# whwu95/MVFNet

Hardware: AMD Instinct MI355X
Metric: clips/sec (fwd+bwd) MVFNet-R50 8x8 224^2 (higher is better)
Workload: dtype bf16; 1 GPU; MVFNet-ResNet50 8x8, 32 clips/GPU of 8x3x224x224, bf16, train step: fwd (batch-stat BN) + loss + bwd + clip + SGD-nesterov; all through the HIP C ABI (stem + 16 bottlenecks + MVF + TSN head); clips_per_gpu=32, frames_per_clip=8, parallelism=dp1: replicas, one flat gradient all-reduce per step

## Files before the change

### include/mvfnet_hip.h

```cpp
#ifndef MVFNET_HIP_H
#define MVFNET_HIP_H

#include <stddef.h>
#include <stdint.h>

#ifdef __cplusplus
extern "C" {
#endif

#define MVF_ABI_VERSION 2

enum { MVF_OK = 0, MVF_EINVAL = -1, MVF_ESHAPE = -2, MVF_EWS = -3, MVF_EHIP = -4, MVF_EUNSUPPORTED = -5 };
enum { MVF_F32 = 0, MVF_BF16 = 1 };
enum { MVF_NCHW = 0, MVF_NHWC = 1 };
enum { MVF_VIEW_T = 1, MVF_VIEW_H = 2, MVF_VIEW_W = 4 };

int mvf_abi_version(void);
const char* mvf_last_error(void);

typedef struct {
    int32_t nt, c, h, w;
    int32_t n_segment;
    int32_t cs;
    int32_t mode;
// ... 158 lines not shown
                          int sums_rows, float* slabs, size_t slab_bytes, int dtype, void* stream);
int mvf_conv1x1_bnbwd_sums_pair(const void* a_in, int a_pitch, const void* w_a, const void* x_in, int x_pitch, const void* w_b, const void* g, int g_pitch,
                                const unsigned char* sign_bits, long m, int c, int k, const float* mean_a, const float* invstd_a, const float* mean_b,
                                const float* invstd_b, float* part_a, float* part_b, int rows, int dtype, void* stream);
int mvf_wgrad_slab_reduce(const float* slabs, int nsplit, int cout, int k, float* dw_oihw, void* stream);
int mvf_maxpool_bn_relu_fwd(const void* z, int n, int h, int w, int c, const float* scale, const float* shift, void* y,
                            unsigned char* argmax, int dtype, void* stream);
int mvf_maxpool_bn_relu_bwd(const unsigned char* argmax, const void* g, int n, int h, int w, int c, void* ga, int dtype,
                            void* stream);
int mvf_maxpool_bwd_sums_rows(int n, int h);
int mvf_maxpool_bn_relu_bwd_apply(const unsigned char* argmax, const void* g, int n, int h, int w, int c, const void* z, const float* gamma,
                                  const float* mean, const float* invstd, const float* scale, const float* shift, const float* dgamma,
                                  const float* dbeta, void* dz, int dtype, void* stream);
int mvf_maxpool_bn_relu_bwd_sums(const unsigned char* argmax, const void* g, int n, int h, int w, int c, void* ga, const void* z, const float* mean,
                                 const float* invstd, const float* scale, const float* shift, float* sums_part, int dtype, void* stream);
int mvf_head_train_fwd(const void* feat, int clips, int t, int hw, int c, const float* fc_w, const float* fc_b, int classes,
                       const long long* labels, const float* drop_mask ,
                       float* pooled, float* scores, float* dscores, float* loss_part, float* loss, int dtype, void* stream);
int mvf_ce_loss(const float* scores, const long long* labels, int clips, int classes, float* dscores, float* loss_part, float* loss,
                void* stream);
int mvf_head_train_bwd(const float* dscores, const float* pooled, const float* fc_w, const float* drop_mask, int clips, int t,
                       int hw, int c, int classes, float* dfc_w, float* dfc_b, float* dpool_ws , void* dfeat, int dtype,
                       void* stream);
size_t mvf_conv2d_wgrad_workspace_bytes(const mvf_conv_desc_t* d);
int mvf_conv2d_nhwc_wgrad(const mvf_conv_desc_t* d, const void* dz, const void* x, const void* x2, int kw_real,
                          int cin_real, int kw_packed, int cin_packed, float* dw_oihw, void* ws, size_t ws_bytes,
                          void* stream);
int mvf_conv2d_nhwc_wgrad_wgs(const mvf_conv_desc_t* d, const void* dz, const void* x, const void* x2, int kw_real,
                              int cin_real, int kw_packed, int cin_packed, float* dw_oihw, void* ws, size_t ws_bytes, int wgs, void* stream);
typedef struct {
// ... 51 lines not shown
```

### mvfnet_amd/_lib.py

```python
import ctypes as C
import os

import torch

_HERE = os.path.dirname(os.path.abspath(__file__))
LIB_PATH = os.environ.get("MVF_LIB_PATH") or os.path.join(_HERE, "libmvfnet_hip.so")

MVF_F32, MVF_BF16 = 0, 1
MVF_NCHW, MVF_NHWC = 0, 1
VIEW_T, VIEW_H, VIEW_W = 1, 2, 4
MODE_BITS = {"T": 1, "TH": 3, "THW": 7}
ERRNAMES = {-1: "MVF_EINVAL", -2: "MVF_ESHAPE", -3: "MVF_EWS", -4: "MVF_EHIP", -5: "MVF_EUNSUPPORTED"}


class MvfDesc(C.Structure):
    _fields_ = [("nt", C.c_int32), ("c", C.c_int32), ("h", C.c_int32), ("w", C.c_int32), ("n_segment", C.c_int32),
                ("cs", C.c_int32), ("mode", C.c_int32), ("layout", C.c_int32), ("dtype", C.c_int32)]


class ConvDesc(C.Structure):
    _fields_ = [("n", C.c_int32), ("h", C.c_int32), ("w", C.c_int32), ("cin", C.c_int32), ("cout", C.c_int32),
                ("kh", C.c_int32), ("kw", C.c_int32), ("stride", C.c_int32), ("pad", C.c_int32),
                ("ho", C.c_int32), ("wo", C.c_int32), ("x_pix_stride", C.c_int32),
                ("dtype", C.c_int32), ("relu", C.c_int32), ("split_c", C.c_int32), ("x2_pix_stride", C.c_int32), ("in_dil", C.c_int32),
# ... 130 lines not shown
    lib.mvf_bn_apply_bits.argtypes = [vp, i64, i32, fp, fp, vp, fp, fp, i32, vp, vp, i32, vp]
    lib.mvf_bn_bwd_apply_masked.restype = i32
    lib.mvf_bn_bwd_apply_masked.argtypes = [vp, i32, vp, vp, i64, i32, fp, fp, fp, fp, fp, fp, fp, i32, vp, i32, vp]
    lib.mvf_bn_bwd_reduce.restype = i32
    lib.mvf_bn_bwd_reduce.argtypes = [vp, i32, vp, vp, i64, i32, fp, fp, fp, fp, i32, vp, fp, fp, vp, sz, i32, vp]
    lib.mvf_bn_bwd_apply.restype = i32
    lib.mvf_bn_bwd_apply.argtypes = [vp, i32, vp, i64, i32, fp, fp, fp, fp, fp, fp, fp, i32, vp, i32, vp]
    lib.mvf_maxpool_bn_relu_fwd.restype = i32
    lib.mvf_maxpool_bn_relu_fwd.argtypes = [vp, i32, i32, i32, i32, fp, fp, vp, vp, i32, vp]
    lib.mvf_maxpool_bn_relu_bwd.restype = i32
    lib.mvf_maxpool_bn_relu_bwd.argtypes = [vp, vp, i32, i32, i32, i32, vp, i32, vp]
    lib.mvf_maxpool_bwd_sums_rows.restype = i32
    lib.mvf_maxpool_bwd_sums_rows.argtypes = [i32, i32]
    lib.mvf_maxpool_bn_relu_bwd_apply.restype = i32
    lib.mvf_maxpool_bn_relu_bwd_apply.argtypes = [vp, vp, i32, i32, i32, i32, vp, fp, fp, fp, fp, fp, fp, fp, vp, i32, vp]
    lib.mvf_maxpool_bn_relu_bwd_sums.restype = i32
    lib.mvf_maxpool_bn_relu_bwd_sums.argtypes = [vp, vp, i32, i32, i32, i32, vp, vp, fp, fp, fp, fp, fp, i32, vp]
    lib.mvf_head_train_fwd.restype = i32
    lib.mvf_head_train_fwd.argtypes = [vp, i32, i32, i32, i32, fp, fp, i32, ll, fp, fp, fp, fp, fp, fp, i32, vp]
    lib.mvf_conv2d_nhwc_fwd_mvf.restype = i32
    lib.mvf_conv2d_nhwc_fwd_mvf.argtypes = [cp, vp, vp, fp, fp, i32, i32, i32, vp, vp, sz, vp]
    lib.mvf_bn_bwd_pair.restype = i32
    lib.mvf_bn_bwd_pair.argtypes = [vp, i32, vp, vp, vp, i64, i32, fp, fp, fp, fp, fp, fp, fp, fp, fp, fp, vp, vp, vp, sz, i32, vp]
    lib.mvf_bn_bwd_wgrad_splits.restype = i32
    lib.mvf_bn_bwd_wgrad_splits.argtypes = [i64, i32, i32, i32, i32]
    lib.mvf_bn_bwd_wgrad_slab_bytes.restype = sz
    lib.mvf_bn_bwd_wgrad_slab_bytes.argtypes = [i64, i32, i32, i32, i32]
    lib.mvf_bn_bwd_apply_wgrad.restype = i32
    lib.mvf_bn_bwd_apply_wgrad.argtypes = [vp, i32, vp, vp, i64, i32, fp, fp, fp, fp, fp, fp, fp, i32, vp, vp, i32, i32, fp, sz, i32, vp]
    lib.mvf_bn_bwd_pair_wgrad.restype = i32
# ... 58 lines not shown
```

### mvfnet_amd/csrc/common.h

```cpp
#pragma once
#include <hip/hip_runtime.h>
#include <stdlib.h>
#include <string.h>
#include <strings.h>
#include <stdint.h>
#include <stdio.h>

#include "mvfnet_hip.h"

void mvf_set_error(const char* fmt, ...);

#define MVF_HIP_OK(call)                                                                        \
    do {                                                                                        \
        hipError_t e__ = (call);                                                                \
        if (e__ != hipSuccess) {                                                                \
            mvf_set_error("%s:%d: %s -> %s", __FILE__, __LINE__, #call, hipGetErrorString(e__)); \
            return MVF_EHIP;                                                                    \
        }                                                                                       \
    } while (0)

#define MVF_REQUIRE(cond, code, ...)    \
    do {                                \
        if (!(cond)) {                  \
            mvf_set_error(__VA_ARGS__); \
// ... 38 lines not shown
                       __uint_as_float(r.y << 16), __uint_as_float(r.y & 0xffff0000u));
}
__device__ __forceinline__ void st4(float* p, float4 v) { *reinterpret_cast<float4*>(p) = v; }
__device__ __forceinline__ void st4(bf16_t* p, float4 v) {
    uint2 r;
    r.x = pack_bf16x2(v.x, v.y);
    r.y = pack_bf16x2(v.z, v.w);
    *reinterpret_cast<uint2*>(p) = r;
}

__device__ __forceinline__ float hswish_f(float u) { return u * fminf(fmaxf(u + 3.0f, 0.0f), 6.0f) * (1.0f / 6.0f); }
__device__ __forceinline__ float hswish_grad_f(float u) {
    float r6 = fminf(fmaxf(u + 3.0f, 0.0f), 6.0f);
    float inner = (u > -3.0f && u < 3.0f) ? 1.0f : 0.0f;
    return r6 * (1.0f / 6.0f) + u * inner * (1.0f / 6.0f);
}

static inline size_t align_up(size_t v, size_t a) { return (v + a - 1) / a * a; }

static inline bool mvf_policy_lookup(const char* name, long* out) {
    const char* p = getenv("MVF_POLICY");
    if (!p) return false;
    const size_t n = strlen(name);
    while (*p) {
        while (*p == ',' || *p == ';' || *p == ' ') ++p;
        const char* e = p;
        while (*e && *e != ',' && *e != ';') ++e;
        const char* eq = (const char*)memchr(p, '=', (size_t)(e - p));
        if (eq && (size_t)(eq - p) == n && strncasecmp(p, name, n) == 0) {
            *out = strtol(eq + 1, nullptr, 10);
// ... 40 lines not shown
    const void* a;
    const void* w;
    const void* g;
    const unsigned char* bits;
    const float* c0;
    const float* c1;
    float* part;
    int rows, mode, M, N, K, xps;
};
struct Wgrad3x3C64Args {
    const void* dz;
    const void* x;
    float* part;
    int N, H, W, xps, nwg;
};
struct WgradStemArgs {
    const void* dz;
    const void* x;
    float* part;
    int N, H, W, Ho, Wo, nwg;
};
namespace mvf_internal {
struct BnBwdWgradArgs {
    const void* g;
    const void* z[2];
    const void* bits;
    const float *gamma[2], *mean[2], *invstd[2], *dgamma[2], *dbeta[2];
    const float *scale, *shift;
    void* dz[2];
    const void* x[2];
    int xps[2];
    float* part[2];
    int g_pitch, M, C, K;
    int rows_per_split, nsplit, ctiles, ktiles;
};
// ... 19 lines not shown
    const float *mean_a, *invstd_a, *mean_b, *invstd_b;
    float *part_a, *part_b;
    int aps, xps, g_pitch, M, rows, rows_per_split, nsplit;
};
int pw_sums_pair_launch(const PwSumsPairArgs& a, hipStream_t st);
int pw_bwd_fused_plan(long m, int c, int k, int* rows_per_split);
int pw_bwd_fused_launch(const PwBwdFusedArgs& a, hipStream_t st);
bool bnbwd_wgrad_tile(int c, int k, int nbn, int mask_mode, int* ct, int* kt);
int bnbwd_wgrad_plan(long m, int c, int k, int nbn, int mask_mode, int* rows_per_split, int* ctiles, int* ktiles);
int bnbwd_wgrad_launch(const BnBwdWgradArgs& a, int nbn, int mask_mode, hipStream_t st);
int wgrad_slab_reduce_launch(const float* part, int nsplit, int cout, int k, float* dw_oihw, hipStream_t st);
bool wgrad3x3_c64_ok(int n, int h, int w, int xps);
int wgrad3x3_c64_wgs(int n, int h);
int wgrad3x3_c64_launch(const Wgrad3x3C64Args& a, hipStream_t st);
bool wgrad_stem_ok(int n, int h, int w, int ho, int wo);
int wgrad_stem_wgs(int n, int ho);
int wgrad_stem_launch(const WgradStemArgs& a, hipStream_t st);
int stem_direct_launch(const StemDirectArgs& a, hipStream_t st);
int conv3x3_c64_launch(const Conv3x3C64Args& a, hipStream_t st);
int pw_sums_launch(const PwSumsArgs& a, hipStream_t st);
}

#ifdef __HIPCC__
typedef int i32x4 __attribute__((ext_vector_type(4)));
__device__ __forceinline__ i32x4 rsrc_words(const void* base, unsigned nbytes) {
    const unsigned long p = (unsigned long)base;
    i32x4 r;
    r.x = __builtin_amdgcn_readfirstlane((int)(unsigned)p);
    r.y = __builtin_amdgcn_readfirstlane((int)((unsigned)(p >> 32) & 0xffffu));
    r.z = __builtin_amdgcn_readfirstlane((int)nbytes);
// ... 13 lines not shown
```

### mvfnet_amd/csrc/train_ops.hip

```cpp
#include <algorithm>
#include <math.h>
#include <stdlib.h>

#include "common.h"

namespace {

constexpr int kThreads = 256;

struct ColPlan {
    int cqb;
    int rl;
    int gx;
    int gy;
    int rows;
};

ColPlan col_plan(long M, int C, int vn = 4, int blocks = 2048) {
    ColPlan p;
    const int cq = C / vn;
    int cqb = 1;
    while (cqb < cq && cqb < 64) cqb <<= 1;
    p.cqb = cqb;
    p.rl = kThreads / cqb;
// ... 901 lines not shown
template <typename ET, int MODE>
__global__ __launch_bounds__(256) void maxpool_bn_bwd_blk_kernel(const unsigned char* amax, const ET* g, int n, int h, int w, int c, int ho, int wo, ET* ga,
                                                                 const ET* z, const float* gamma, const float* mean, const float* invstd, const float* scale,
                                                                 const float* shift, const float* dgamma, const float* dbeta, float inv_m, float* part, int nblk,
                                                                 ET* dz) {
    constexpr int VC = 16 / (int)sizeof(ET);
    __shared__ float red[MODE == 0 ? 256 * 2 * VC : 1];
    const int ncg = c / VC, hw2 = w >> 1, hb = h >> 1;
    const int cq = threadIdx.x % ncg;
    float scv[VC], shv[VC], muv[VC], k1[VC], k2[VC], k3[VC];
#pragma unroll
    for (int j = 0; j < VC; ++j) {
        const int ch = cq * VC + j;
        scv[j] = scale[ch]; shv[j] = shift[ch]; muv[j] = mean[ch];
        if constexpr (MODE == 0) { k1[j] = invstd[ch]; k2[j] = 0.f; k3[j] = 0.f; }
        else { k1[j] = gamma[ch] * invstd[ch]; k2[j] = dbeta[ch] * inv_m; k3[j] = invstd[ch] * dgamma[ch] * inv_m; }
    }
    float s1[VC], s2[VC];
#pragma unroll
    for (int j = 0; j < VC; ++j) { s1[j] = 0.f; s2[j] = 0.f; }
    auto ldv = [](const ET* p, float (&f)[VC]) {
        const uint4 u = *reinterpret_cast<const uint4*>(p);
        if constexpr (sizeof(ET) == 4) {
            f[0] = __uint_as_float(u.x); f[1] = __uint_as_float(u.y); f[2] = __uint_as_float(u.z); f[3] = __uint_as_float(u.w);
        } else {
            f[0] = __uint_as_float(u.x << 16); f[1] = __uint_as_float(u.x & 0xffff0000u); f[2] = __uint_as_float(u.y << 16); f[3] = __uint_as_float(u.y & 0xffff0000u);
            f[4] = __uint_as_float(u.z << 16); f[5] = __uint_as_float(u.z & 0xffff0000u); f[6] = __uint_as_float(u.w << 16); f[7] = __uint_as_float(u.w & 0xffff0000u);
        }
    };
    auto stv = [](ET* p, const float (&f)[VC]) {
        uint4 u;
// ... 29 lines not shown
#pragma unroll
                for (int j = 0; j < 4; ++j) am[k][j] = (unsigned char)(a4 >> (8 * j));
            }
            ldv(g + oidx, gv[k]);
        }
        long zi[4];
#pragma unroll
        for (int p = 0; p < 4; ++p) {
            zi[p] = (((long)img * h + 2 * bh + (p >> 1)) * w + 2 * bw + (p & 1)) * c + cq * VC;
            ldv(z + zi[p], zv[p]);
        }
#pragma unroll
        for (int p = 0; p < 4; ++p) {
            const int a = p >> 1, b = p & 1;
            float acc[VC];
#pragma unroll
            for (int j = 0; j < VC; ++j) acc[j] = 0.f;
#pragma unroll
            for (int k = 0; k < 4; ++k) {
                const int wi = k >> 1, wj = k & 1;
                if ((wi == 1 && a == 0) || (wj == 1 && b == 0)) continue;
                const unsigned me = (unsigned)(a + 1 - 2 * wi) * 3u + (unsigned)(b + 1 - 2 * wj);
#pragma unroll
                for (int j = 0; j < VC; ++j)
                    if (okw[k] && am[k][j] == me) acc[j] += gv[k][j];
            }
            if constexpr (MODE == 0) {
                if (ga) stv(ga + zi[p], acc);
            }
            if constexpr (sizeof(ET) == 2) {
#pragma unroll
                for (int j = 0; j < VC; ++j) acc[j] = bf16_to_f32(f32_to_bf16(acc[j]));
            }
            if constexpr (MODE == 0) {
#pragma unroll
                for (int j = 0; j < VC; ++j) {
                    const float gm = (zv[p][j] * scv[j] + shv[j]) > 0.f ? acc[j] : 0.f;
                    s1[j] += gm;
                    s2[j] += gm * ((zv[p][j] - muv[j]) * k1[j]);
                }
            } else {
                float o[VC];
#pragma unroll
                for (int j = 0; j < VC; ++j) {
                    const float gm = (zv[p][j] * scv[j] + shv[j]) > 0.f ? acc[j] : 0.f;
                    o[j] = k1[j] * (gm - k2[j] - (zv[p][j] - muv[j]) * k3[j]);
                }
                stv(dz + zi[p], o);
            }
        }
    }
    if constexpr (MODE == 0) {
#pragma unroll
        for (int j = 0; j < VC; ++j) {
            red[(2 * j) * 256 + threadIdx.x] = s1[j];
            red[(2 * j + 1) * 256 + threadIdx.x] = s2[j];
        }
        __syncthreads();
        if ((int)threadIdx.x < c) {
            const int q = threadIdx.x / VC, j = threadIdx.x - q * VC;
            float a = 0.f, b = 0.f;
            for (int t = q; t < 256; t += ncg) {
// ... 826 lines not shown
```

### mvfnet_amd/csrc/wgrad_nhwc.hip

```cpp
#include <algorithm>

#include <stdlib.h>

#include "common.h"

namespace {

constexpr int kThreads = 256;
constexpr int BMR = 32;
typedef float f32x16 __attribute__((ext_vector_type(16)));

struct WgArgs {
    const void* dz;
    const void* x;
    const void* x2;
    float* part;
    int N, H, W, Cin, Cout, KH, KW, stride, pad, Ho, Wo, xps, split_c, x2ps;
    int M, K, rows_per_split, tiles_k;
    int tiles, nsplit;
    unsigned fd_hw_mul, fd_hw_shr, fd_w_mul, fd_w_shr;
    int xcd_rr;
    int abl;
};

// ... 1242 lines not shown
    return launch_wgrad_reduce(a.part, nsplit, d->cout, cin_real, kh_p, kw_real, kw_packed, cin_packed, dw_oihw, st);
}
extern "C" {

int mvf_conv2d_nhwc_wgrad(const mvf_conv_desc_t* d, const void* dz, const void* x, const void* x2, int kw_real, int cin_real,
                          int kw_packed, int cin_packed, float* dw_oihw, void* ws, size_t ws_bytes, void* stream) {
    return wgrad_impl(d, dz, x, x2, kw_real, cin_real, kw_packed, cin_packed, dw_oihw, ws, ws_bytes, stream, 0);
}

int mvf_conv2d_nhwc_wgrad_wgs(const mvf_conv_desc_t* d, const void* dz, const void* x, const void* x2, int kw_real, int cin_real,
                              int kw_packed, int cin_packed, float* dw_oihw, void* ws, size_t ws_bytes, int wgs, void* stream) {
    MVF_REQUIRE(wgs >= 8 && wgs <= 4096, MVF_EINVAL, "wgrad_wgs: wgs=%d outside 8 .. 4096", wgs);
    return wgrad_impl(d, dz, x, x2, kw_real, cin_real, kw_packed, cin_packed, dw_oihw, ws, ws_bytes, stream, wgs);
}

int mvf_pack_conv_weights_batched(const mvf_pack_job_t* jobs_dev, int njobs, int total_blocks, int dtype, void* stream) {
    MVF_REQUIRE(jobs_dev && njobs > 0 && total_blocks > 0 && (dtype == MVF_F32 || dtype == MVF_BF16), MVF_EINVAL, "pack_conv_weights_batched: bad argument");
    if (dtype == MVF_F32)
        hipLaunchKernelGGL(pack_batched_kernel<float>, dim3(total_blocks), dim3(256), 0, (hipStream_t)stream, jobs_dev, njobs);
    else
        hipLaunchKernelGGL(pack_batched_kernel<bf16_t>, dim3(total_blocks), dim3(256), 0, (hipStream_t)stream, jobs_dev, njobs);
    MVF_LAUNCH_CHECK();
    return MVF_OK;
}

int mvf_pack_conv_weight_dgrad(const float* w_oihw, int cout, int cin, int kh, int kw, void* w_packed, int dtype, void* stream) {
    MVF_REQUIRE(w_oihw && w_packed && cout > 0 && cin > 0 && kh > 0 && kw > 0, MVF_EINVAL, "pack_conv_weight_dgrad: bad argument");
    const long total = (long)cout * cin * kh * kw;
    const int blocks = (int)std::min<long>((total + 255) / 256, 4096);
    if (dtype == MVF_F32)
// ... 9 lines not shown
```

### mvfnet_amd/csrc/wgrad_stem.hip

```cpp
#include <algorithm>
#include <stdlib.h>

#include "common.h"

namespace {

typedef float f32x16 __attribute__((ext_vector_type(16)));
typedef short bf16x8_t __attribute__((ext_vector_type(8)));

struct KArgs {
    const char* dz;
    const char* x;
    float* part;
    int N, H, W, Ho, Wo;
    int bands_per_frame, bands;
    int rowb;
    int xbytes, dpix;
    int ksr;
    unsigned fd_bpf_mul, fd_bpf_shr, fd_ksr_mul, fd_ksr_shr;
};

__device__ __forceinline__ int fdiv(int n, unsigned mul, unsigned shr) { return (int)((__umulhi((unsigned)n, mul) + (unsigned)n) >> shr); }
__device__ __forceinline__ int swzf(int pixel) { return ((pixel >> 1) & 1) << 2; }

template <int kR>
__global__ __launch_bounds__(256, 2) void wgrad_stem_kernel(KArgs a) {
    extern __shared__ __attribute__((aligned(16))) char smem[];
    char* Xs = smem;
    char* Ds = smem + (a.xbytes + 1023) / 1024 * 1024;
    const int tid = threadIdx.x, lane = tid & 63;
    const int wave = __builtin_amdgcn_readfirstlane(tid >> 6);
    const int wm = wave & 1, kg = wave >> 1;
    constexpr unsigned kOOB = 0x80000000u;
    const i32x4 gs_x = rsrc_words(a.x, (unsigned)((long)a.N * a.H * a.rowb));
    const i32x4 gs_d = rsrc_words(a.dz, (unsigned)((long)a.N * a.Ho * a.Wo * 128));
    const unsigned lds_x = (unsigned)__builtin_amdgcn_readfirstlane((int)(unsigned)(size_t)(__attribute__((address_space(3))) char*)Xs);
    const unsigned lds_d = (unsigned)__builtin_amdgcn_readfirstlane((int)(unsigned)(size_t)(__attribute__((address_space(3))) char*)Ds);
    const int nx = (a.xbytes + 1023) >> 10, nd = a.dpix >> 3;
    const int lp = lane >> 3, lu = lane & 7;

    const int tg = lane >> 4, ti = lane & 15;
    const int trow = (ti >> 2) + 8 * (tg >> 1);
    const int tunit = 2 * (tg & 1) + ((ti & 3) >> 1), thalf = ti & 1;
    const int offA = trow * 128 + (((wm * 4 + tunit) ^ swzf(trow)) << 4) + thalf * 8;
// ... 3 lines not shown
    auto gather = [&](const char* lo_p, const char* hi_p) {
        const v4s lo = __builtin_amdgcn_ds_read_tr16_b64_v4i16((lds_v4s)(lo_p));
        const v4s hi = __builtin_amdgcn_ds_read_tr16_b64_v4i16((lds_v4s)(hi_p));
        bf16x8_t v;
        v[0] = lo[0]; v[1] = lo[1]; v[2] = lo[2]; v[3] = lo[3];
        v[4] = hi[0]; v[5] = hi[1]; v[6] = hi[2]; v[7] = hi[3];
        return v;
    };

    f32x16 acc[4];
#pragma unroll
    for (int t = 0; t < 4; ++t)
#pragma unroll
        for (int r = 0; r < 16; ++r) acc[t][r] = 0.f;

    const int nks = a.dpix >> 4;
    for (int b = blockIdx.x; b < a.bands; b += gridDim.x) {
        const int img = fdiv(b, a.fd_bpf_mul, a.fd_bpf_shr);
        const int oh0 = (b - img * a.bands_per_frame) * kR;
        __syncthreads();
        {
            const long xbase = ((long)img * a.H + 2 * oh0) * a.rowb;
            for (int i = wave; i < nx; i += 4) {
                const int o = i * 1024 + lane * 16;
                glds16(gs_x, lds_x + (unsigned)(i * 1024), o < a.xbytes ? (unsigned)(xbase + o) : kOOB);
            }
            const long dbase = ((long)img * a.Ho + oh0) * a.Wo * 128;
            for (int i = wave; i < nd; i += 4) {
                const int p = i * 8 + lp;
                glds16(gs_d, lds_d + (unsigned)(i * 1024), (unsigned)(dbase + p * 128 + ((lu ^ swzf(p)) << 4)));
            }
        }
        asm volatile("s_waitcnt vmcnt(0)" ::: "memory");
        __syncthreads();
        for (int ks = 0; ks < nks; ++ks) {
            const int r = fdiv(ks, a.fd_ksr_mul, a.fd_ksr_shr), ow0 = (ks - r * a.ksr) * 16;
            const bf16x8_t fa = gather(Ds + ks * 2048 + offA, Ds + ks * 2048 + offA + 4 * 128);
            const char* xb = Xs + (2 * r + 4 * kg) * a.rowb + ow0 * 16 + offB;
            bf16x8_t fb[4];
#pragma unroll
            for (int t = 0; t < 4; ++t) {
                if (t < 3 || kg == 0) fb[t] = gather(xb + t * a.rowb, xb + t * a.rowb + 64);
            }
#pragma unroll
            for (int t = 0; t < 4; ++t) {
                if (t < 3 || kg == 0) acc[t] = __builtin_amdgcn_mfma_f32_32x32x16_bf16(fa, fb[t], acc[t], 0, 0, 0);
            }
        }
// ... 1 lines not shown
    const int lr = lane >> 5, lc = lane & 31;
    float* out = a.part + (long)blockIdx.x * 64 * 224;
#pragma unroll
    for (int t = 0; t < 4; ++t) {
        if (t < 3 || kg == 0) {
            const int col = (4 * kg + t) * 32 + lc;
#pragma unroll
            for (int r = 0; r < 16; ++r) {
                const int row = wm * 32 + (r & 3) + 8 * (r >> 2) + 4 * lr;
                out[row * 224 + col] = acc[t][r];
            }
        }
    }
}

inline void fd_make(unsigned d, unsigned& mul, unsigned& shr) {
    unsigned l = 0;
    while ((1ull << l) < d) ++l;
    mul = (unsigned)((((1ull << l) - d) << 32) / d + 1);
    shr = l;
}

static int band_rows() {
    static const int r = mvf_policy_int("wgrad_stem_r", 2);
    return r == 1 ? 1 : 2;
}

}

namespace mvf_internal {

bool wgrad_stem_ok(int n, int h, int w, int ho, int wo) {
    static const bool on = (mvf_policy_int("wgrad_stem_direct", 1) != 0);
    return on && n > 0 && wo >= 16 && wo % 16 == 0 && ho % 2 == 0 && (w * 8) % 16 == 0 && 2 * (ho - 1) + 6 < h && 2 * (wo - 1) + 7 < w &&
           (long)n * h * w * 8 < 0x7ffffff0L && (long)n * ho * wo * 128 < 0x7ffffff0L &&
           (2 * 2 + 5) * w * 8 + 1024 + 2 * wo * 128 <= 72 * 1024;
}

int wgrad_stem_wgs(int n, int ho) {
    static const int env = std::max(1, mvf_policy_int("wgrad_stem_wgs", 768));
    return (int)std::min<long>(env, (long)n * (ho / band_rows()));
}

int wgrad_stem_launch(const WgradStemArgs& w, hipStream_t st) {
    KArgs a = {};
    a.dz = (const char*)w.dz; a.x = (const char*)w.x; a.part = w.part;
    a.N = w.N; a.H = w.H; a.W = w.W; a.Ho = w.Ho; a.Wo = w.Wo;
    const int kR = band_rows();
    a.bands_per_frame = w.Ho / kR;
    a.bands = w.N * a.bands_per_frame;
    a.rowb = w.W * 8;
    a.xbytes = (2 * kR + 5) * a.rowb;
    a.dpix = kR * w.Wo;
    a.ksr = w.Wo / 16;
    fd_make((unsigned)a.bands_per_frame, a.fd_bpf_mul, a.fd_bpf_shr);
    fd_make((unsigned)a.ksr, a.fd_ksr_mul, a.fd_ksr_shr);
    const int lds = (a.xbytes + 1023) / 1024 * 1024 + a.dpix * 128;
    static bool attr = false;
    if (!attr) {
        MVF_HIP_OK(hipFuncSetAttribute((const void*)wgrad_stem_kernel<1>, hipFuncAttributeMaxDynamicSharedMemorySize, 72 * 1024));
        MVF_HIP_OK(hipFuncSetAttribute((const void*)wgrad_stem_kernel<2>, hipFuncAttributeMaxDynamicSharedMemorySize, 72 * 1024));
        attr = true;
    }
    if (kR == 1) hipLaunchKernelGGL(wgrad_stem_kernel<1>, dim3(w.nwg), dim3(256), lds, st, a);
    else hipLaunchKernelGGL(wgrad_stem_kernel<2>, dim3(w.nwg), dim3(256), lds, st, a);
    MVF_LAUNCH_CHECK();
    return MVF_OK;
}

}
```

### mvfnet_amd/train_engine.py

```python
import ctypes as C
import os

import torch

from . import _lib
from ._lib import ConvDesc, MvfDesc, check, lib

F32 = _lib.MVF_F32

_ConvDescT, _MvfDescT = ConvDesc, MvfDesc
_DESC_CACHE = {}


def ConvDesc(*a):
    d = _DESC_CACHE.get(a)
    if d is None:
        d = _DESC_CACHE[a] = _ConvDescT(*a)
    return d


def MvfDesc(*a):
    k = ("mvf",) + a
    d = _DESC_CACHE.get(k)
    if d is None:
# ... 173 lines not shown

    def _reduce(self, g, g_pitch, z, m, eng, mask_mode, ymask, gm_out):
        ws = eng.workspace(lib.mvf_bn_workspace_bytes(m, self.c))
        check(lib.mvf_bn_bwd_reduce(_p(g), g_pitch, _p(z), _p(ymask), m, self.c, _p(self.mean), _p(self.invstd), _p(self.scale),
                                    _p(self.shift), mask_mode, _p(gm_out), _p(self.dgamma), _p(self.dbeta), _p(ws), ws.numel(), eng.dt, _st()),
              "mvf_bn_bwd_reduce")

    def _apply_bwd(self, g, g_pitch, z, m, eng, mask_mode, ymask, gm_out):
        src, pitch, mode = (gm_out, self.c, 0) if gm_out is not None else (g, g_pitch, mask_mode)
        dz = eng.buf((id(self), "dz"), z.shape, z.dtype)
        sg, sb = (self._zero, self._zero) if self.frozen else (self.dgamma, self.dbeta)
        check(lib.mvf_bn_bwd_apply_masked(_p(src), pitch, _p(z), _p(ymask) if mode in (1, 4) else None, m, self.c, _p(self.gamma), _p(self.mean),
                                          _p(self.invstd), _p(self.scale), _p(self.shift), _p(sg), _p(sb), mode, _p(dz), eng.dt,
                                          _st()), "mvf_bn_bwd_apply")
        return dz


class _TConv(object):

    def __init__(self, conv, eng, stem=False):
        self.eng = eng
        self.w = conv.weight
        self.dw = eng.grad_of(conv.weight)
        self.cout, self.cin, self.kh, self.kw = conv.weight.shape
        self.stride, self.pad = conv.stride[0], conv.padding[0]
        self.stem = stem
        dev = conv.weight.device
        td = eng.tdtype
        if stem:
            self.wp = torch.empty(self.cout, self.kh, 8, 4, device=dev, dtype=td)
# ... 117 lines not shown
                                                  _p(bn.dgamma), _p(bn.dbeta), _p(dz), _p(ws), ws.numel(), _st()), "conv + bn backward apply")

    def launch_fwd_apply(self, d, x, bn, residual, rbn, out, bits, ws):
        check(lib.mvf_conv2d_nhwc_fwd_bnapply(C.byref(d), _p(x), None, _p(self.wp), _p(bn.scale), _p(bn.shift), _p(residual),
                                              _p(rbn.scale if rbn else None), _p(rbn.shift if rbn else None), _p(out), _p(bits),
                                              _p(ws), ws.numel(), _st()), "conv fwd + bn apply")

    def launch_fwd(self, d, x, x2, z, ws, part, shift):
        if part is None:
            check(lib.mvf_conv2d_nhwc_fwd_ws(C.byref(d), _p(x), _p(x2), _p(self.wp), None, None, _p(z), _p(ws), ws.numel(), _st()), "conv fwd")
        else:
            check(lib.mvf_conv2d_nhwc_fwd_stats(C.byref(d), _p(x), _p(x2), _p(self.wp), _p(z), _p(part), _p(shift), _p(ws), ws.numel(), _st()),
                  "conv fwd+stats")

    def wgrad(self, dz, x, n, h, w, ho, wo, eng, x_pitch=None, x2=None, split_c=0, on_main=False):
        d = self.desc(n, h, w, ho, wo, x_pitch or self.cin, split_c)
        kwr, cinr, kwp, cinp = (self.kw, self.cin, 8, 4) if self.stem else (self.kw, self.cin, self.kw, self.cin)
        nbytes = lib.mvf_conv2d_wgrad_workspace_bytes(C.byref(d))
        side = None if on_main else eng.side_stream()
        if side is None:
            ws = eng.workspace(nbytes)
            check(lib.mvf_conv2d_nhwc_wgrad(C.byref(d), _p(dz), _p(x), _p(x2), kwr, cinr, kwp, cinp, _p(self.dw), _p(ws), ws.numel(), _st()), "conv wgrad")
            return
        ws = eng.workspace(nbytes, side=True)

        def launch():
            check(lib.mvf_conv2d_nhwc_wgrad(C.byref(d), _p(dz), _p(x), _p(x2), kwr, cinr, kwp, cinp, _p(self.dw), _p(ws), ws.numel(), _st()), "conv wgrad")
        eng.on_side(launch)

    def fuses_wgrad(self, eng, m, c, mask_mode, nbn=1):
# ... 985 lines not shown
                                     _p(self.dfc_w), _p(self.dfc_b), _p(dpool), _p(g), self.dt, _st()), "head bwd")
        gated = sums = False
        for i in range(len(self.blocks) - 1, -1, -1):
            req = self.blocks[i - 1].wants_gated_gradient(self) if i > 0 else None
            g = self.blocks[i].backward(g, nt, self, g_gated=gated, gate=req, sums_done=sums)
            gated, sums = self.blocks[i].gated_out, self.blocks[i].sums_out
            if i == self._tail_block:
                self._launch_tail_allreduce()
        ho, wo = s["ho"], s["wo"]
        bn = self.stem_bn
        rows = lib.mvf_maxpool_bwd_sums_rows(nt, ho)
        part = self.buf("stem_bnsums", (64, rows, 2), torch.float32)
        check(lib.mvf_maxpool_bn_relu_bwd_sums(_p(s["amax"]), _p(g), nt, ho, wo, 64, None, _p(s["z0"]), _p(bn.mean), _p(bn.invstd),
                                               _p(bn.scale), _p(bn.shift), _p(part), self.dt, _st()), "maxpool bwd + bn sums")
        check(lib.mvf_bn_bwd_finalize(_p(part), rows, 64, _p(bn.dgamma), _p(bn.dbeta), _st()), "bn bwd finalize")
        dz0 = self.buf((id(bn), "dz"), s["z0"].shape, s["z0"].dtype)
        sg, sb = (bn._zero, bn._zero) if bn.frozen else (bn.dgamma, bn.dbeta)
        check(lib.mvf_maxpool_bn_relu_bwd_apply(_p(s["amax"]), _p(g), nt, ho, wo, 64, _p(s["z0"]), _p(bn.gamma), _p(bn.mean), _p(bn.invstd), _p(bn.scale),
                                                _p(bn.shift), _p(sg), _p(sb), _p(dz0), self.dt, _st()), "maxpool bwd + bn apply")
        self.flush_side()
        self.stem.wgrad(dz0, s["xp"], nt, s["hp"], s["wp"], ho, wo, self, on_main=True)
        self.join_side()
        if self.keep_io:
            self.io = dict(p0=self.buf("p0", (g.shape[0], 64)), g_p0=g, gfeat=self.buf("gfeat", tuple(s["feat_shape"])), nt=nt, b=b, t=t)
        self.saved = None

    exchange_enabled = True

    def _ddp_active(self):
        import torch.distributed as dist
        return self.exchange_enabled and dist.is_available() and dist.is_initialized() and (dist.get_world_size() > 1 or self.force_allreduce)

    overlap_allreduce = _policy("ddp_overlap", 1) != 0

# ... 121 lines not shown
```

Baseline: 1795 clips/s.

## Fuse stem maxpool/BN backward apply into the stem weight-gradient kernel

The stem's maxpool+BN+ReLU backward apply is folded into the stem wgrad kernel. Each band loads the pre-BN activation z0 into LDS, then gathers pooled gradients and argmax, computes dz in place in LDS, and runs the wgrad GEMM on it. This removes a separate apply launch and the round trip of writing and re-reading the full-resolution dz0 tensor. In exchange the kernel does extra per-band gather work, uses more LDS for per-channel coefficients, and raises its launch-bounds occupancy target, with a fallback to the two-launch path when the shape or alignment checks fail.

```diff
diff --git a/include/mvfnet_hip.h b/include/mvfnet_hip.h
--- a/include/mvfnet_hip.h
+++ b/include/mvfnet_hip.h
@@ -196,6 +196,11 @@
                                   const float* dbeta, void* dz, int dtype, void* stream);
 int mvf_maxpool_bn_relu_bwd_sums(const unsigned char* argmax, const void* g, int n, int h, int w, int c, void* ga, const void* z, const float* mean,
                                  const float* invstd, const float* scale, const float* shift, float* sums_part, int dtype, void* stream);
+size_t mvf_stem_bwd_apply_wgrad_workspace_bytes(int n, int hp, int wp, int ho, int wo, int dtype);
+int mvf_stem_bwd_apply_wgrad_plan(int n, int hp, int wp, int ho, int wo, int dtype, int force);
+int mvf_stem_bwd_apply_wgrad(const unsigned char* argmax, const void* g, const void* z0, int n, int ho, int wo, const float* gamma, const float* mean,
+                             const float* invstd, const float* scale, const float* shift, const float* dgamma, const float* dbeta, const void* xp, int hp, int wp,
+                             float* dw_oihw, void* dz0, void* ws, size_t ws_bytes, int force, int dtype, void* stream);
 int mvf_head_train_fwd(const void* feat, int clips, int t, int hw, int c, const float* fc_w, const float* fc_b, int classes,
                        const long long* labels, const float* drop_mask ,
                        float* pooled, float* scores, float* dscores, float* loss_part, float* loss, int dtype, void* stream);
diff --git a/mvfnet_amd/_lib.py b/mvfnet_amd/_lib.py
--- a/mvfnet_amd/_lib.py
+++ b/mvfnet_amd/_lib.py
@@ -168,6 +168,12 @@
     lib.mvf_maxpool_bwd_sums_rows.argtypes = [i32, i32]
     lib.mvf_maxpool_bn_relu_bwd_apply.restype = i32
     lib.mvf_maxpool_bn_relu_bwd_apply.argtypes = [vp, vp, i32, i32, i32, i32, vp, fp, fp, fp, fp, fp, fp, fp, vp, i32, vp]
+    lib.mvf_stem_bwd_apply_wgrad_workspace_bytes.restype = C.c_size_t
+    lib.mvf_stem_bwd_apply_wgrad_workspace_bytes.argtypes = [i32, i32, i32, i32, i32, i32]
+    lib.mvf_stem_bwd_apply_wgrad_plan.restype = i32
+    lib.mvf_stem_bwd_apply_wgrad_plan.argtypes = [i32, i32, i32, i32, i32, i32, i32]
+    lib.mvf_stem_bwd_apply_wgrad.restype = i32
+    lib.mvf_stem_bwd_apply_wgrad.argtypes = [vp, vp, vp, i32, i32, i32, fp, fp, fp, fp, fp, fp, fp, vp, i32, i32, fp, vp, vp, C.c_size_t, i32, i32, vp]
     lib.mvf_maxpool_bn_relu_bwd_sums.restype = i32
     lib.mvf_maxpool_bn_relu_bwd_sums.argtypes = [vp, vp, i32, i32, i32, i32, vp, vp, fp, fp, fp, fp, fp, i32, vp]
     lib.mvf_head_train_fwd.restype = i32
diff --git a/mvfnet_amd/csrc/common.h b/mvfnet_amd/csrc/common.h
--- a/mvfnet_amd/csrc/common.h
+++ b/mvfnet_amd/csrc/common.h
@@ -76,6 +76,40 @@
     float r6 = fminf(fmaxf(u + 3.0f, 0.0f), 6.0f);
     float inner = (u > -3.0f && u < 3.0f) ? 1.0f : 0.0f;
     return r6 * (1.0f / 6.0f) + u * inner * (1.0f / 6.0f);
+}
+
+template <int VC, bool kRound>
+__device__ __forceinline__ void pool_blk_gather(int a, int b, const bool (&okw)[4], const unsigned char (&am)[4][VC], const float (&gv)[4][VC], float (&acc)[VC]) {
+#pragma unroll
+    for (int j = 0; j < VC; ++j) acc[j] = 0.f;
+#pragma unroll
+    for (int k = 0; k < 4; ++k) {
+        const int wi = k >> 1, wj = k & 1;
+        if ((wi == 1 && a == 0) || (wj == 1 && b == 0)) continue;
+        const unsigned me = (unsigned)(a + 1 - 2 * wi) * 3u + (unsigned)(b + 1 - 2 * wj);
+#pragma unroll
+        for (int j = 0; j < VC; ++j)
+            if (okw[k] && am[k][j] == me) acc[j] += gv[k][j];
+    }
+    if constexpr (kRound) {
+#pragma unroll
+        for (int j = 0; j < VC; ++j) acc[j] = bf16_to_f32(f32_to_bf16(acc[j]));
+    }
+}
+__device__ __forceinline__ float pool_bn_gate(float z, float acc, float scale, float shift) { return (z * scale + shift) > 0.f ? acc : 0.f; }
+__device__ __forceinline__ float pool_bn_bwd_dz(float z, float acc, float scale, float shift, float mean, float k1, float k2, float k3) {
+    const float gm = pool_bn_gate(z, acc, scale, shift);
+    return k1 * (gm - k2 - (z - mean) * k3);
+}
+__device__ __forceinline__ void pool_bn_bwd_coefs(float gamma, float invstd, float dgamma, float dbeta, float inv_m, float& k1, float& k2, float& k3) {
+    k1 = gamma * invstd; k2 = dbeta * inv_m; k3 = invstd * dgamma * inv_m;
+}
+__device__ __forceinline__ void unpack_bf16x8(const uint4 u, float (&f)[8]) {
+    f[0] = __uint_as_float(u.x << 16); f[1] = __uint_as_float(u.x & 0xffff0000u); f[2] = __uint_as_float(u.y << 16); f[3] = __uint_as_float(u.y & 0xffff0000u);
+    f[4] = __uint_as_float(u.z << 16); f[5] = __uint_as_float(u.z & 0xffff0000u); f[6] = __uint_as_float(u.w << 16); f[7] = __uint_as_float(u.w & 0xffff0000u);
+}
+__device__ __forceinline__ uint4 pack_bf16x8(const float (&f)[8]) {
+    return make_uint4(pack_bf16x2(f[0], f[1]), pack_bf16x2(f[2], f[3]), pack_bf16x2(f[4], f[5]), pack_bf16x2(f[6], f[7]));
 }
 
 static inline size_t align_up(size_t v, size_t a) { return (v + a - 1) / a * a; }
@@ -146,11 +180,18 @@
     float* part;
     int N, H, W, xps, nwg;
 };
+struct StemBwdApplyArgs {
+    const unsigned char* amax;
+    const void* g;
+    const float *gamma, *mean, *invstd, *scale, *shift, *dgamma, *dbeta;
+    float inv_m;
+};
 struct WgradStemArgs {
     const void* dz;
     const void* x;
     float* part;
     int N, H, W, Ho, Wo, nwg;
+    const StemBwdApplyArgs* apply;
 };
 namespace mvf_internal {
 struct BnBwdWgradArgs {
@@ -200,6 +241,7 @@
 int wgrad3x3_c64_wgs(int n, int h);
 int wgrad3x3_c64_launch(const Wgrad3x3C64Args& a, hipStream_t st);
 bool wgrad_stem_ok(int n, int h, int w, int ho, int wo);
+bool wgrad_stem_fused_ok(int n, int h, int w, int ho, int wo);
 int wgrad_stem_wgs(int n, int ho);
 int wgrad_stem_launch(const WgradStemArgs& a, hipStream_t st);
 int stem_direct_launch(const StemDirectArgs& a, hipStream_t st);
diff --git a/mvfnet_amd/csrc/train_ops.hip b/mvfnet_amd/csrc/train_ops.hip
--- a/mvfnet_amd/csrc/train_ops.hip
+++ b/mvfnet_amd/csrc/train_ops.hip
@@ -939,7 +939,7 @@
         const int ch = cq * VC + j;
         scv[j] = scale[ch]; shv[j] = shift[ch]; muv[j] = mean[ch];
         if constexpr (MODE == 0) { k1[j] = invstd[ch]; k2[j] = 0.f; k3[j] = 0.f; }
-        else { k1[j] = gamma[ch] * invstd[ch]; k2[j] = dbeta[ch] * inv_m; k3[j] = invstd[ch] * dgamma[ch] * inv_m; }
+        else pool_bn_bwd_coefs(gamma[ch], invstd[ch], dgamma[ch], dbeta[ch], inv_m, k1[j], k2[j], k3[j]);
     }
     float s1[VC], s2[VC];
 #pragma unroll
@@ -999,38 +999,24 @@
         for (int p = 0; p < 4; ++p) {
             const int a = p >> 1, b = p & 1;
             float acc[VC];
-#pragma unroll
-            for (int j = 0; j < VC; ++j) acc[j] = 0.f;
-#pragma unroll
-            for (int k = 0; k < 4; ++k) {
-                const int wi = k >> 1, wj = k & 1;
-                if ((wi == 1 && a == 0) || (wj == 1 && b == 0)) continue;
-                const unsigned me = (unsigned)(a + 1 - 2 * wi) * 3u + (unsigned)(b + 1 - 2 * wj);
-#pragma unroll
-                for (int j = 0; j < VC; ++j)
-                    if (okw[k] && am[k][j] == me) acc[j] += gv[k][j];
-            }
             if constexpr (MODE == 0) {
+                pool_blk_gather<VC, false>(a, b, okw, am, gv, acc);
                 if (ga) stv(ga + zi[p], acc);
-            }
-            if constexpr (sizeof(ET) == 2) {
-#pragma unroll
-                for (int j = 0; j < VC; ++j) acc[j] = bf16_to_f32(f32_to_bf16(acc[j]));
-            }
-            if constexpr (MODE == 0) {
+                if constexpr (sizeof(ET) == 2) {
+#pragma unroll
+                    for (int j = 0; j < VC; ++j) acc[j] = bf16_to_f32(f32_to_bf16(acc[j]));
+                }
 #pragma unroll
                 for (int j = 0; j < VC; ++j) {
-                    const float gm = (zv[p][j] * scv[j] + shv[j]) > 0.f ? acc[j] : 0.f;
+                    const float gm = pool_bn_gate(zv[p][j], acc[j], scv[j], shv[j]);
                     s1[j] += gm;
                     s2[j] += gm * ((zv[p][j] - muv[j]) * k1[j]);
                 }
             } else {
+                pool_blk_gather<VC, sizeof(ET) == 2>(a, b, okw, am, gv, acc);
                 float o[VC];
 #pragma unroll
-                for (int j = 0; j < VC; ++j) {
-                    const float gm = (zv[p][j] * scv[j] + shv[j]) > 0.f ? acc[j] : 0.f;
-                    o[j] = k1[j] * (gm - k2[j] - (zv[p][j] - muv[j]) * k3[j]);
-                }
+                for (int j = 0; j < VC; ++j) o[j] = pool_bn_bwd_dz(zv[p][j], acc[j], scv[j], shv[j], muv[j], k1[j], k2[j], k3[j]);
                 stv(dz + zi[p], o);
             }
         }
diff --git a/mvfnet_amd/csrc/wgrad_nhwc.hip b/mvfnet_amd/csrc/wgrad_nhwc.hip
--- a/mvfnet_amd/csrc/wgrad_nhwc.hip
+++ b/mvfnet_amd/csrc/wgrad_nhwc.hip
@@ -1280,6 +1280,47 @@
     return wgrad_impl(d, dz, x, x2, kw_real, cin_real, kw_packed, cin_packed, dw_oihw, ws, ws_bytes, stream, wgs);
 }
 
+static mvf_conv_desc_t stem_wgrad_desc(int n, int hp, int wp, int ho, int wo, int dtype) {
+    mvf_conv_desc_t d = {};
+    d.n = n; d.h = hp; d.w = wp; d.cin = 32; d.cout = 64; d.kh = 7; d.kw = 1; d.stride = 2; d.pad = 0; d.ho = ho; d.wo = wo; d.x_pix_stride = 4; d.dtype = dtype;
+    return d;
+}
+static bool stem_bwd_fused_shape(const mvf_conv_desc_t* d, int force) {
+    static const int on = mvf_policy_int("stem_bwd_fused", 1);
+    return (force < 0 ? on : force) != 0 && wg_direct_stem(d) && mvf_internal::wgrad_stem_fused_ok(d->n, d->h, d->w, d->ho, d->wo);
+}
+
+size_t mvf_stem_bwd_apply_wgrad_workspace_bytes(int n, int hp, int wp, int ho, int wo, int dtype) {
+    const mvf_conv_desc_t d = stem_wgrad_desc(n, hp, wp, ho, wo, dtype);
+    return mvf_conv2d_wgrad_workspace_bytes(&d);
+}
+
+int mvf_stem_bwd_apply_wgrad_plan(int n, int hp, int wp, int ho, int wo, int dtype, int force) {
+    const mvf_conv_desc_t d = stem_wgrad_desc(n, hp, wp, ho, wo, dtype);
+    return n > 0 && ho > 0 && wo > 0 && stem_bwd_fused_shape(&d, force) ? 1 : 0;
+}
+
+int mvf_stem_bwd_apply_wgrad(const unsigned char* argmax, const void* g, const void* z0, int n, int ho, int wo, const float* gamma, const float* mean,
+                             const float* invstd, const float* scale, const float* shift, const float* dgamma, const float* dbeta, const void* xp, int hp, int wp,
+                             float* dw_oihw, void* dz0, void* ws, size_t ws_bytes, int force, int dtype, void* stream) {
+    MVF_REQUIRE(argmax && g && z0 && gamma && mean && invstd && scale && shift && dgamma && dbeta && xp && dw_oihw && n > 0 && ho > 0 && wo > 0 && hp > 0 && wp > 0,
+                MVF_EINVAL, "stem_bwd_apply_wgrad: bad argument");
+    MVF_REQUIRE(dtype == MVF_F32 || dtype == MVF_BF16, MVF_EINVAL, "stem_bwd_apply_wgrad: bad dtype");
+    const mvf_conv_desc_t d = stem_wgrad_desc(n, hp, wp, ho, wo, dtype);
+    MVF_REQUIRE(ws && ws_bytes >= mvf_conv2d_wgrad_workspace_bytes(&d), MVF_EWS, "stem_bwd_apply_wgrad: workspace too small");
+    if (stem_bwd_fused_shape(&d, force) && ((uintptr_t)z0 | (uintptr_t)xp | (uintptr_t)g) % 16 == 0 && (uintptr_t)argmax % 8 == 0) {
+        const StemBwdApplyArgs f = {argmax, g, gamma, mean, invstd, scale, shift, dgamma, dbeta, 1.0f / (float)((long)n * ho * wo)};
+        WgradStemArgs w = {z0, xp, (float*)ws, n, hp, wp, ho, wo, mvf_internal::wgrad_stem_wgs(n, ho), &f};
+        const int rc = mvf_internal::wgrad_stem_launch(w, (hipStream_t)stream);
+        if (rc != MVF_OK) return rc;
+        return launch_wgrad_reduce((const float*)ws, w.nwg, 64, 3, 7, 7, 8, 4, dw_oihw, (hipStream_t)stream);
+    }
+    MVF_REQUIRE(dz0, MVF_EINVAL, "stem_bwd_apply_wgrad: the two-launch path needs the dz0 buffer");
+    const int rc = mvf_maxpool_bn_relu_bwd_apply(argmax, g, n, ho, wo, 64, z0, gamma, mean, invstd, scale, shift, dgamma, dbeta, dz0, dtype, stream);
+    if (rc != MVF_OK) return rc;
+    return wgrad_impl(&d, dz0, xp, nullptr, 7, 3, 8, 4, dw_oihw, ws, ws_bytes, stream, 0);
+}
+
 int mvf_pack_conv_weights_batched(const mvf_pack_job_t* jobs_dev, int njobs, int total_blocks, int dtype, void* stream) {
     MVF_REQUIRE(jobs_dev && njobs > 0 && total_blocks > 0 && (dtype == MVF_F32 || dtype == MVF_BF16), MVF_EINVAL, "pack_conv_weights_batched: bad argument");
     if (dtype == MVF_F32)
diff --git a/mvfnet_amd/csrc/wgrad_stem.hip b/mvfnet_amd/csrc/wgrad_stem.hip
--- a/mvfnet_amd/csrc/wgrad_stem.hip
+++ b/mvfnet_amd/csrc/wgrad_stem.hip
@@ -18,16 +18,22 @@
     int xbytes, dpix;
     int ksr;
     unsigned fd_bpf_mul, fd_bpf_shr, fd_ksr_mul, fd_ksr_shr;
+    const unsigned char* amax;
+    const char* g;
+    const float *gamma, *mean, *invstd, *scale, *shift, *dgamma, *dbeta;
+    float inv_m;
 };
 
 __device__ __forceinline__ int fdiv(int n, unsigned mul, unsigned shr) { return (int)((__umulhi((unsigned)n, mul) + (unsigned)n) >> shr); }
 __device__ __forceinline__ int swzf(int pixel) { return ((pixel >> 1) & 1) << 2; }
 
-template <int kR>
-__global__ __launch_bounds__(256, 2) void wgrad_stem_kernel(KArgs a) {
+template <int kR, bool kFuse>
+__global__ __launch_bounds__(256, kFuse ? 3 : 2) void wgrad_stem_kernel(KArgs a) {
+    static_assert(!kFuse || kR == 2, "the fused form walks rows of 2 x 2 pixel blocks");
     extern __shared__ __attribute__((aligned(16))) char smem[];
     char* Xs = smem;
     char* Ds = smem + (a.xbytes + 1023) / 1024 * 1024;
+    float* Cs = reinterpret_cast<float*>(Ds + a.dpix * 128);
     const int tid = threadIdx.x, lane = tid & 63;
     const int wave = __builtin_amdgcn_readfirstlane(tid >> 6);
     const int wm = wave & 1, kg = wave >> 1;
@@ -61,6 +67,63 @@
 #pragma unroll
         for (int r = 0; r < 16; ++r) acc[t][r] = 0.f;
 
+    struct PoolWin { uint4 g[4]; uint2 am[4]; };
+    const int hp = a.Ho >> 1, wp = a.Wo >> 1, items = a.Wo * 4, cq = tid & 7;
+    auto load_win = [&](int i, int img, int bh, PoolWin& w) {
+        const int bw = i >> 3;
+#pragma unroll
+        for (int k = 0; k < 4; ++k) {
+            const long oidx = (((long)img * hp + min(bh + (k >> 1), hp - 1)) * wp + min(bw + (k & 1), wp - 1)) * 64 + cq * 8;
+            w.am[k] = *reinterpret_cast<const uint2*>(a.amax + oidx);
+            w.g[k] = *reinterpret_cast<const uint4*>(a.g + oidx * 2);
+        }
+    };
+    auto apply_win = [&](int i, int bh, const PoolWin& w) {
+        const int bw = i >> 3;
+        bool okw[4];
+#pragma unroll
+        for (int k = 0; k < 4; ++k) okw[k] = bh + (k >> 1) < hp && bw + (k & 1) < wp;
+#pragma unroll 1
+        for (int h = 0; h < 2; ++h) {
+            unsigned char am[4][4];
+            float gv[4][4];
+#pragma unroll
+            for (int k = 0; k < 4; ++k) {
+                const unsigned a4 = h ? w.am[k].y : w.am[k].x, g0 = h ? w.g[k].z : w.g[k].x, g1 = h ? w.g[k].w : w.g[k].y;
+#pragma unroll
+                for (int j = 0; j < 4; ++j) am[k][j] = (unsigned char)(a4 >> (8 * j));
+                gv[k][0] = __uint_as_float(g0 << 16); gv[k][1] = __uint_as_float(g0 & 0xffff0000u);
+                gv[k][2] = __uint_as_float(g1 << 16); gv[k][3] = __uint_as_float(g1 & 0xffff0000u);
+            }
+            float cf[6][4];
+#pragma unroll
+            for (int t = 0; t < 6; ++t) {
+                const float4 c4 = *reinterpret_cast<const float4*>(Cs + t * 64 + cq * 8 + h * 4);
+                cf[t][0] = c4.x; cf[t][1] = c4.y; cf[t][2] = c4.z; cf[t][3] = c4.w;
+            }
+#pragma unroll
+            for (int p = 0; p < 4; ++p) {
+                const int px = (p >> 1) * a.Wo + 2 * bw + (p & 1);
+                uint2* q = reinterpret_cast<uint2*>(Ds + px * 128 + ((cq ^ swzf(px)) << 4) + h * 8);
+                const uint2 zu = *q;
+                const float zv[4] = {__uint_as_float(zu.x << 16), __uint_as_float(zu.x & 0xffff0000u), __uint_as_float(zu.y << 16), __uint_as_float(zu.y & 0xffff0000u)};
+                float acc[4], o[4];
+                pool_blk_gather<4, true>(p >> 1, p & 1, okw, am, gv, acc);
+#pragma unroll
+                for (int j = 0; j < 4; ++j) o[j] = pool_bn_bwd_dz(zv[j], acc[j], cf[0][j], cf[1][j], cf[2][j], cf[3][j], cf[4][j], cf[5][j]);
+                *q = make_uint2(pack_bf16x2(o[0], o[1]), pack_bf16x2(o[2], o[3]));
+            }
+        }
+    };
+    if constexpr (kFuse) {
+        if (tid < 64) {
+            float k1, k2, k3;
+            pool_bn_bwd_coefs(a.gamma[tid], a.invstd[tid], a.dgamma[tid], a.dbeta[tid], a.inv_m, k1, k2, k3);
+            Cs[tid] = a.scale[tid]; Cs[64 + tid] = a.shift[tid]; Cs[128 + tid] = a.mean[tid];
+            Cs[192 + tid] = k1; Cs[256 + tid] = k2; Cs[320 + tid] = k3;
+        }
+    }
+
     const int nks = a.dpix >> 4;
     for (int b = blockIdx.x; b < a.bands; b += gridDim.x) {
         const int img = fdiv(b, a.fd_bpf_mul, a.fd_bpf_shr);
@@ -78,7 +141,20 @@
                 glds16(gs_d, lds_d + (unsigned)(i * 1024), (unsigned)(dbase + p * 128 + ((lu ^ swzf(p)) << 4)));
             }
         }
-        asm volatile("s_waitcnt vmcnt(0)" ::: "memory");
+        if constexpr (kFuse) {
+            const int bh = oh0 >> 1;
+            PoolWin w0;
+            if (tid < items) load_win(tid, img, bh, w0);
+            asm volatile("s_waitcnt vmcnt(0)" ::: "memory");
+            __syncthreads();
+            if (tid < items) apply_win(tid, bh, w0);
+            for (int i = tid + 256; i < items; i += 256) {
+                load_win(i, img, bh, w0);
+                apply_win(i, bh, w0);
+            }
+        } else {
+            asm volatile("s_waitcnt vmcnt(0)" ::: "memory");
+        }
         __syncthreads();
         for (int ks = 0; ks < nks; ++ks) {
             const int r = fdiv(ks, a.fd_ksr_mul, a.fd_ksr_shr), ow0 = (ks - r * a.ksr) * 16;
@@ -110,6 +186,8 @@
     }
 }
 
+constexpr int kFuseCoefBytes = 6 * 64 * 4;
+
 inline void fd_make(unsigned d, unsigned& mul, unsigned& shr) {
     unsigned l = 0;
     while ((1ull << l) < d) ++l;
@@ -131,6 +209,11 @@
     return on && n > 0 && wo >= 16 && wo % 16 == 0 && ho % 2 == 0 && (w * 8) % 16 == 0 && 2 * (ho - 1) + 6 < h && 2 * (wo - 1) + 7 < w &&
            (long)n * h * w * 8 < 0x7ffffff0L && (long)n * ho * wo * 128 < 0x7ffffff0L &&
            (2 * 2 + 5) * w * 8 + 1024 + 2 * wo * 128 <= 72 * 1024;
+}
+
+bool wgrad_stem_fused_ok(int n, int h, int w, int ho, int wo) {
+    return wgrad_stem_ok(n, h, w, ho, wo) && band_rows() == 2 && (2 * 2 + 5) * w * 8 + 1024 + 2 * wo * 128 + kFuseCoefBytes <= 72 * 1024 &&
+           (long)n * (ho / 2) * (wo / 2) * 128 < 0x7ffffff0L;
 }
 
 int wgrad_stem_wgs(int n, int ho) {
@@ -151,15 +234,24 @@
     a.ksr = w.Wo / 16;
     fd_make((unsigned)a.bands_per_frame, a.fd_bpf_mul, a.fd_bpf_shr);
     fd_make((unsigned)a.ksr, a.fd_ksr_mul, a.fd_ksr_shr);
-    const int lds = (a.xbytes + 1023) / 1024 * 1024 + a.dpix * 128;
+    const StemBwdApplyArgs* f = w.apply;
+    MVF_REQUIRE(!f || wgrad_stem_fused_ok(w.N, w.H, w.W, w.Ho, w.Wo), MVF_EUNSUPPORTED, "wgrad_stem: the fused form does not take this shape");
+    if (f) {
+        a.amax = f->amax; a.g = (const char*)f->g;
+        a.gamma = f->gamma; a.mean = f->mean; a.invstd = f->invstd; a.scale = f->scale; a.shift = f->shift; a.dgamma = f->dgamma; a.dbeta = f->dbeta;
+        a.inv_m = f->inv_m;
+    }
+    const int lds = (a.xbytes + 1023) / 1024 * 1024 + a.dpix * 128 + (f ? kFuseCoefBytes : 0);
     static bool attr = false;
     if (!attr) {
-        MVF_HIP_OK(hipFuncSetAttribute((const void*)wgrad_stem_kernel<1>, hipFuncAttributeMaxDynamicSharedMemorySize, 72 * 1024));
-        MVF_HIP_OK(hipFuncSetAttribute((const void*)wgrad_stem_kernel<2>, hipFuncAttributeMaxDynamicSharedMemorySize, 72 * 1024));
+        MVF_HIP_OK(hipFuncSetAttribute((const void*)wgrad_stem_kernel<1, false>, hipFuncAttributeMaxDynamicSharedMemorySize, 72 * 1024));
+        MVF_HIP_OK(hipFuncSetAttribute((const void*)wgrad_stem_kernel<2, false>, hipFuncAttributeMaxDynamicSharedMemorySize, 72 * 1024));
+        MVF_HIP_OK(hipFuncSetAttribute((const void*)wgrad_stem_kernel<2, true>, hipFuncAttributeMaxDynamicSharedMemorySize, 72 * 1024));
         attr = true;
     }
-    if (kR == 1) hipLaunchKernelGGL(wgrad_stem_kernel<1>, dim3(w.nwg), dim3(256), lds, st, a);
-    else hipLaunchKernelGGL(wgrad_stem_kernel<2>, dim3(w.nwg), dim3(256), lds, st, a);
+    if (f) hipLaunchKernelGGL((wgrad_stem_kernel<2, true>), dim3(w.nwg), dim3(256), lds, st, a);
+    else if (kR == 1) hipLaunchKernelGGL((wgrad_stem_kernel<1, false>), dim3(w.nwg), dim3(256), lds, st, a);
+    else hipLaunchKernelGGL((wgrad_stem_kernel<2, false>), dim3(w.nwg), dim3(256), lds, st, a);
     MVF_LAUNCH_CHECK();
     return MVF_OK;
 }
diff --git a/mvfnet_amd/train_engine.py b/mvfnet_amd/train_engine.py
--- a/mvfnet_amd/train_engine.py
+++ b/mvfnet_amd/train_engine.py
@@ -211,6 +211,12 @@
                                           _p(self.invstd), _p(self.scale), _p(self.shift), _p(sg), _p(sb), mode, _p(dz), eng.dt,
                                           _st()), "mvf_bn_bwd_apply")
         return dz
+
+
+class _StemDz(object):
+
+    def __init__(self, amax, g, z0, bn, dgamma, dbeta):
+        self.amax, self.g, self.z0, self.bn, self.dgamma, self.dbeta = amax, g, z0, bn, dgamma, dbeta
 
 
 class _TConv(object):
@@ -358,6 +364,13 @@
                   "conv fwd+stats")
 
     def wgrad(self, dz, x, n, h, w, ho, wo, eng, x_pitch=None, x2=None, split_c=0, on_main=False):
+        if isinstance(dz, _StemDz):
+            f, bn = dz, dz.bn
+            ws = eng.workspace(lib.mvf_stem_bwd_apply_wgrad_workspace_bytes(n, h, w, ho, wo, eng.dt))
+            check(lib.mvf_stem_bwd_apply_wgrad(_p(f.amax), _p(f.g), _p(f.z0), n, ho, wo, _p(bn.gamma), _p(bn.mean), _p(bn.invstd), _p(bn.scale), _p(bn.shift),
+                                               _p(f.dgamma), _p(f.dbeta), _p(x), h, w, _p(self.dw), None, _p(ws), ws.numel(), -1, eng.dt, _st()),
+                  "stem bwd apply + wgrad")
+            return
         d = self.desc(n, h, w, ho, wo, x_pitch or self.cin, split_c)
         kwr, cinr, kwp, cinp = (self.kw, self.cin, 8, 4) if self.stem else (self.kw, self.cin, self.kw, self.cin)
         nbytes = lib.mvf_conv2d_wgrad_workspace_bytes(C.byref(d))
@@ -1373,10 +1386,13 @@
         check(lib.mvf_maxpool_bn_relu_bwd_sums(_p(s["amax"]), _p(g), nt, ho, wo, 64, None, _p(s["z0"]), _p(bn.mean), _p(bn.invstd),
                                                _p(bn.scale), _p(bn.shift), _p(part), self.dt, _st()), "maxpool bwd + bn sums")
         check(lib.mvf_bn_bwd_finalize(_p(part), rows, 64, _p(bn.dgamma), _p(bn.dbeta), _st()), "bn bwd finalize")
-        dz0 = self.buf((id(bn), "dz"), s["z0"].shape, s["z0"].dtype)
         sg, sb = (bn._zero, bn._zero) if bn.frozen else (bn.dgamma, bn.dbeta)
-        check(lib.mvf_maxpool_bn_relu_bwd_apply(_p(s["amax"]), _p(g), nt, ho, wo, 64, _p(s["z0"]), _p(bn.gamma), _p(bn.mean), _p(bn.invstd), _p(bn.scale),
-                                                _p(bn.shift), _p(sg), _p(sb), _p(dz0), self.dt, _st()), "maxpool bwd + bn apply")
+        if lib.mvf_stem_bwd_apply_wgrad_plan(nt, s["hp"], s["wp"], ho, wo, self.dt, -1):
+            dz0 = _StemDz(s["amax"], g, s["z0"], bn, sg, sb)
+        else:
+            dz0 = self.buf((id(bn), "dz"), s["z0"].shape, s["z0"].dtype)
+            check(lib.mvf_maxpool_bn_relu_bwd_apply(_p(s["amax"]), _p(g), nt, ho, wo, 64, _p(s["z0"]), _p(bn.gamma), _p(bn.mean), _p(bn.invstd), _p(bn.scale),
+                                                    _p(bn.shift), _p(sg), _p(sb), _p(dz0), self.dt, _st()), "maxpool bwd + bn apply")
         self.flush_side()
         self.stem.wgrad(dz0, s["xp"], nt, s["hp"], s["wp"], ho, wo, self, on_main=True)
         self.join_side()
```

After: 1784 clips/s. About the same (-0.6%).
